# TianyiFranklinWang/MIRROR

Hardware: AMD Instinct MI355X
Metric: SSL samples/sec (slide+RNA pairs) (higher is better)
Workload: dtype bf16; 1 GPU; BASELINE c2: B=16/GPU x [4096 patch tokens x 1024-d] + [2048 genes], D=512, RNA depth 6 / 8 heads, train mode, local-batch InfoNCE; precision_policy=bf16, per_gpu_batch=16, global_batch=16, parallelism=dp1, grad_bucket_dtype=f32, step_launch=hip_graph

## Files before the change

### mirror_amd/csrc/gemm_big.hip

```cpp
#include "gemm_kernel.h"

static thread_local GemmTail g_tail = {nullptr, nullptr, 0, 0, 0, 0, 0, 0, 0, 0, 0.f};
GemmTail* gemm_pending_tail() { return &g_tail; }

namespace {

constexpr int BIG = 256, NTB = 512, BWM = 4, BWN = 2;

__device__ __forceinline__ f32x4 round_bf16_4(f32x4 x) {
    return f32x4{bf2f(f2bf(x[0])), bf2f(f2bf(x[1])), bf2f(f2bf(x[2])), bf2f(f2bf(x[3]))};
}
struct TileRow { int b0, t0, row0; };
template <int EPI>
__device__ __forceinline__ f32x4 epi_quad(const GemmArgs& g, f32x4 x, int grow, int gcol, const TileRow& tr) {
    if constexpr (EPI == MH_EPI_MASKPOS) {
        x = round_bf16_4(x);
        const int rpb = g.epi.rows_per_batch, first = g.epi.first;
        int t = tr.t0 + (grow - tr.row0), b = tr.b0;
        if (t >= rpb) { t -= rpb; b += 1; }
        if (t >= first && g.epi.mask[(long)b * (rpb - first) + (t - first)] != 0.f) x = *reinterpret_cast<const f32x4*>(g.epi.token + gcol);
        return x + *reinterpret_cast<const f32x4*>(g.epi.pos + (long)t * g.N + gcol);
    } else {
        return x;
    }
// ... 960 lines not shown
    __shared__ f32x4 red[PS > 1 ? 256 : 1];
    const int ql = threadIdx.x % QB, pg = threadIdx.x / QB;
    const long quads = mn / 4;
    for (long qb = blockIdx.x; qb * QB < quads; qb += gridDim.x) {
        const long q = qb * QB + ql;
        const bool live = q < quads;
        const long i = q * 4, r = live ? i / N : 0, c = live ? i % N : 0;
        f32x4 s = {0.f, 0.f, 0.f, 0.f};
        if (live) {
            int p = pg;
            for (; p + 7 * PS < parts; p += 8 * PS) {
                f32x4 v[8];
#pragma unroll
                for (int u = 0; u < 8; u++) v[u] = ld4_bf16(P + (long)(p + u * PS) * mn + i);
#pragma unroll
                for (int u = 0; u < 8; u++) s += v[u];
            }
            for (; p < parts; p += PS) s += ld4_bf16(P + (long)p * mn + i);
            if constexpr (TAIL) {
                f32x4 acc = {0.f, 0.f, 0.f, 0.f};
                const int total = t.batch * t.KT;
                auto ld = [&](int k, float& a, f32x4& b) {
                    const int z = k / t.KT, kk = k - z * t.KT;
                    const long ia = z * t.sA + (long)kk * t.lda + r, ib = z * t.sB + (long)kk * t.ldb + c;
                    a = t.a_f32 ? reinterpret_cast<const float*>(t.A)[ia] : bf2f(reinterpret_cast<const bf16_t*>(t.A)[ia]);
                    if (t.b_f32) b = *reinterpret_cast<const f32x4*>(reinterpret_cast<const float*>(t.B) + ib);
                    else {
                        const u32x2 w = *reinterpret_cast<const u32x2*>(reinterpret_cast<const bf16_t*>(t.B) + ib);
                        b = f32x4{__uint_as_float(w[0] << 16), __uint_as_float(w[0] & 0xffff0000u), __uint_as_float(w[1] << 16), __uint_as_float(w[1] & 0xffff0000u)};
                    }
                };
                int k = pg;
                for (; k + 7 * PS < total; k += 8 * PS) {
                    float a[8];
                    f32x4 b[8];
#pragma unroll
                    for (int u = 0; u < 8; u++) ld(k + u * PS, a[u], b[u]);
#pragma unroll
                    for (int u = 0; u < 8; u++) acc += b[u] * a[u];
                }
                for (; k < total; k += PS) {
                    float a;
                    f32x4 b;
                    ld(k, a, b);
                    acc += b * a;
                }
                s += acc * t.alpha;
            }
        }
        if constexpr (PS > 1) {
            __syncthreads();
            red[threadIdx.x] = s;
            __syncthreads();
            if (pg == 0 && live) {
#pragma unroll
                for (int u = 1; u < PS; u++) s += red[u * QB + ql];
            }
        }
        if (pg == 0 && live) {
            f32x4* cp = reinterpret_cast<f32x4*>(C + r * ldc + c);
            *cp = *cp + s;
        }
    }
}
static void launch_fold(const float* ws_, int parts, long mn, float* C, long ldc, int N, hipStream_t s) {
#ifdef MH_EXP
    if (getenv("MH_EXP_SKIP_FOLD")) { g_tail.KT = 0; return; }
#endif
    const bf16_t* ws = reinterpret_cast<const bf16_t*>(ws_);
    const long blocks1 = mh_cdiv(mn / 4, 256);
    const bool tail = g_tail.KT > 0 && (g_tail.ldb % 4) == 0 && (g_tail.sB % 4) == 0 && ((uintptr_t)g_tail.B & (g_tail.b_f32 ? 15 : 7)) == 0;
    const bool share = tail && blocks1 < 1024;
    const dim3 grid((unsigned)min(share ? mh_cdiv(mn / 4, 64) : blocks1, share ? 4096L : 2048L));
#define FOLD_(TAIL, PS) hipLaunchKernelGGL((fold_partials_kernel<TAIL, PS>), grid, dim3(256), 0, s, ws, parts, mn, C, ldc, N, g_tail)
    if (tail) {
        if (share) FOLD_(true, 4); else FOLD_(true, 1);
        g_tail.KT = 0;
    } else {
        FOLD_(false, 1);
    }
#undef FOLD_
}

static int pq_grid(long units) {
    static const int cus = [] { hipDeviceProp_t p; int d = 0; (void)hipGetDevice(&d); return hipGetDeviceProperties(&p, d) == hipSuccess ? p.multiProcessorCount : 256; }();
    return (int)(units < cus ? units : cus);
}
static int pq_variant(const GemmArgs& a, bool bf16_tiles, bool part, int epi) {
    const bool relu = a.act == MH_ACT_RELU;
    if (part) return a.alpha == 1.f ? 0 : 1;
    if (bf16_tiles) {
        if (a.accumulate || (epi != 0 && relu)) return -1;
        return relu ? 2 : (a.alpha == 1.f && !a.bias ? 0 : 1);
    }
    if (a.atomic || (epi != 0 && (relu || a.accumulate))) return -1;
    return a.accumulate ? (relu ? -1 : 2) : (relu ? 1 : 0);
}
template <typename K>
static void pp_attr(K kern) {
    (void)hipFuncSetAttribute(reinterpret_cast<const void*>(kern), hipFuncAttributeMaxDynamicSharedMemorySize, PP_LDS);
}
#define PQ_LAUNCH_VAR_(TC, AKC, BKC, PART, EPI, VAR, s, a, units_, grid)                                  \
    do {                                                                                             \
        static const bool attrq_ = (pp_attr(gemm_pq_kernel<TC, AKC, BKC, PART, EPI, VAR>), true);    \
        (void)attrq_;                                                                                \
        hipLaunchKernelGGL((gemm_pq_kernel<TC, AKC, BKC, PART, EPI, VAR>), dim3(pq_grid(units_)), dim3(NTB), PQ_LDS, s, a, (int)units_, \
                           (int)(grid).x, (int)(grid).y);                                            \
    } while (0)
#define PP_LAUNCH_(TC, AKC, BKC, PART, EPI, grid, s, a)                                              \
    do {                                                                                             \
        const int var_ = pq_variant(a, sizeof(TC) == 2, PART, EPI);                                  \
        const bool pq_ = !(a).shared_chip && var_ >= 0;                                              \
        gemm_note_variant("%s<%s,%s,%s%s%s>", pq_ ? "gemm_pq_kernel" : "gemm_pp_kernel", gemm_tn<TC>(), \
                          gemm_tf(AKC), gemm_tf(BKC), (PART) ? ",part" : "", (EPI) == 0 ? "" : ((EPI) == 1 ? ",epi1" : ((EPI) == 2 ? ",epi2" : ",epi3"))); \
        if (pq_) {                                                                                   \
            const long units_ = (long)(grid).x * (grid).y * (grid).z;                                \
            if (var_ == 0) PQ_LAUNCH_VAR_(TC, AKC, BKC, PART, EPI, 0, s, a, units_, grid);           \
            else if (var_ == 1) PQ_LAUNCH_VAR_(TC, AKC, BKC, PART, EPI, 1, s, a, units_, grid);      \
            else if constexpr ((EPI) == 0 && !(PART)) PQ_LAUNCH_VAR_(TC, AKC, BKC, PART, EPI, 2, s, a, units_, grid); \
        } else {                                                                                     \
            static const bool attr_ = (pp_attr(gemm_pp_kernel<TC, AKC, BKC, PART, EPI>), true);      \
            (void)attr_;                                                                             \
            hipLaunchKernelGGL((gemm_pp_kernel<TC, AKC, BKC, PART, EPI>), grid, dim3(NTB), PP_LDS, s, a); \
        }                                                                                            \
    } while (0)

template <typename TC>
void launch_big(GemmArgs& a, int akc, int bkc, int batch, hipStream_t s) {
    a.tiles_m = (a.M + BIG - 1) / BIG;
    a.tiles_n = a.N / BIG;
    dim3 grid(a.tiles_m * a.tiles_n, a.split_k, batch);
    const long parts = (long)a.split_k * batch, mn = (long)a.M * a.N;
    const bool partial = a.atomic && a.ws && a.M % BIG == 0 && a.ws_floats * 2 >= parts * mn && ((uintptr_t)a.ws & 15) == 0 && a.vecC &&
                         a.sC1 == 0 && a.sC2 == 0 && parts >= 8;
    if (!partial) a.ws = nullptr;
#define PP_DISPATCH_(PART)                                                             \
    do {                                                                               \
        if (akc && bkc) PP_LAUNCH_(TC, true, true, PART, 0, grid, s, a);               \
        else if (akc) PP_LAUNCH_(TC, true, false, PART, 0, grid, s, a);                \
        else if (bkc) PP_LAUNCH_(TC, false, true, PART, 0, grid, s, a);                \
        else PP_LAUNCH_(TC, false, false, PART, 0, grid, s, a);                        \
    } while (0)
    if constexpr (sizeof(TC) == 4) {
        if (partial) {
            PP_DISPATCH_(true);
            launch_fold((const float*)a.ws, (int)parts, mn, (float*)a.C, (long)a.ldc, a.N, s);
            return;
        }
    }
    PP_DISPATCH_(false);
#undef PP_DISPATCH_
}

}

bool gemm_try_big_fp8(GemmArgs& a, int dtC, int batch, hipStream_t s) {
    const bool ok = a.M > BIG && a.N % BIG == 0 && a.K % 64 == 0 && a.k_per_split == a.K && a.split_k == 1 && !a.atomic && !a.accumulate &&
                    a.vecA && a.vecB && a.vecC && !a.R && a.diag == 0.f && a.scale_a && a.scale_b;
    if (!ok || (long)((a.M + BIG - 1) / BIG) * (a.N / BIG) * batch < 128) return false;
    a.tiles_m = (a.M + BIG - 1) / BIG;
    a.tiles_n = a.N / BIG;
    dim3 grid(a.tiles_m * a.tiles_n, 1, batch);
    gemm_note_variant("gemm_big_kernel<%s,true,true,fp8>", dtC == MH_BF16 ? "bf16" : "float");
    if (dtC == MH_BF16) hipLaunchKernelGGL((gemm_big_kernel<bf16_t>), grid, dim3(NTB), 0, s, a);
    else hipLaunchKernelGGL((gemm_big_kernel<float>), grid, dim3(NTB), 0, s, a);
    return true;
}

const char* gemm_big_epi(GemmArgs& a, int akc, int bkc, int dtC, int batch, hipStream_t s) {
    if (!(akc && a.M > BIG && a.N % BIG == 0 && a.K % 64 == 0 && a.split_k == 1 && a.k_per_split == a.K && !a.atomic && !a.accumulate && !a.R &&
          a.diag == 0.f && a.vecA && a.vecB && a.vecC && batch == 1))
        return "shape is not on the 256 x 256 kernel (K-contiguous bf16 A, M > 256, N % 256 == 0, K % 64 == 0, one batch, no split-K / accumulate / R / diag)";
    if (a.a_rpb != 0 && a.a_rpb < BIG) return "a_rows_per_batch must be >= 256";
    if (a.ldc != a.N) return "C must be contiguous (ldc == N)";
    const mh_gemm_epi& e = a.epi;
    a.tiles_m = (a.M + BIG - 1) / BIG;
    a.tiles_n = a.N / BIG;
    dim3 grid(a.tiles_m * a.tiles_n, 1, 1);
#define EPI_LAUNCH_(TC, EPI) \
    do { if (bkc) PP_LAUNCH_(TC, true, true, false, EPI, grid, s, a); else PP_LAUNCH_(TC, true, false, false, EPI, grid, s, a); } while (0)
    switch (e.kind) {
    case MH_EPI_DROPADD:
        if (dtC != MH_F32 || !e.resid || !(e.p >= 0.f && e.p < 1.f) || (e.offset & 7) || ((uintptr_t)e.resid & 15)) return "DROPADD: f32 C, a 16-byte aligned residual, 0 <= p < 1, offset % 8 == 0";
        EPI_LAUNCH_(float, MH_EPI_DROPADD);
        return nullptr;
    case MH_EPI_MASKPOS:
        if (dtC != MH_F32 || !e.mask || !e.token || !e.pos || e.rows_per_batch < BIG || e.first < 0) return "MASKPOS: f32 C, mask / token / pos, rows_per_batch >= 256";
        if (((uintptr_t)e.token & 15) || ((uintptr_t)e.pos & 15)) return "MASKPOS: token / pos must be 16-byte aligned";
        EPI_LAUNCH_(float, MH_EPI_MASKPOS);
        return nullptr;
    case MH_EPI_SQERR:
        if (dtC != MH_BF16 || !e.mask || !e.tgt || !e.sq || e.rows_per_batch <= 0 || e.rows_per_batch % BIG || a.M % e.rows_per_batch || a.act != MH_ACT_NONE) return "SQERR: bf16 C, mask / tgt / sq, rows_per_batch % 256 == 0";
        if (((uintptr_t)e.tgt & 15) || e.tgt_bs % 4) return "SQERR: tgt must be 16-byte aligned";
        EPI_LAUNCH_(bf16_t, MH_EPI_SQERR);
        return nullptr;
// ... 32 lines not shown
```

### mirror_amd/functional.py

```python
from __future__ import annotations

from dataclasses import dataclass
from typing import List, Optional, Tuple

import os

import torch
from torch.autograd import Function

from . import kernels as K
from ._lib import ACT_NONE, ACT_RELU, MH_BF16, MH_F32

f32, bf16 = torch.float32, torch.bfloat16


@dataclass(frozen=True)
class Precision:
    name: str
    mma: int
    act: torch.dtype
    pinv_mma: int
    fp8_fwd: bool = False


# ... 1542 lines not shown
        dz_new = K.gemm(dz, tr(T3), alpha=0.25, mma=pm, out_dtype=f32)
        dP = K.gemm(dT3, tr(T2), alpha=-1.0, mma=pm, out_dtype=f32)
        dT2 = K.gemm(tr(P), dT3, alpha=-1.0, mma=pm, out_dtype=f32)
        K.gemm(dT2, tr(P), out=dP, accumulate=True, R=dT2, rcoef=-7.0, mma=pm)
        K.gemm(tr(P), dT2, out=dP, accumulate=True, mma=pm)
        K.gemm(dP, tr(z), out=dX, accumulate=True, mma=pm)
        K.gemm(tr(a2), dP, out=dz_new, accumulate=True, mma=pm)
        dz = dz_new
    z0 = saved[0][0]
    K.pinv_z0_bwd(a2, K.cast(z0, f32), dz, st, dX)
    return dX


def pinv_forward_tile(a2: torch.Tensor, iters: int, want_a2b: bool = False):
    st = K.pinv_absmax(a2, zeros((4,), a2.device).view(torch.int64))
    a2b = K.cast(a2, bf16)
    zs = torch.empty((iters + 1,) + tuple(a2.shape), device=a2.device, dtype=bf16)
    pt = torch.empty((iters, 2) + tuple(a2.shape), device=a2.device, dtype=bf16)
    K.cast(K.pinv_z0(a2, st), bf16, out=zs[0])
    saved = []
    for k in range(iters):
        z, P, T2 = zs[k], pt[k, 1], pt[k, 0]
        K.gemm(a2b, z, P, mma=MH_BF16)
        K.gemm(P, P, T2, diag=15.0, R=P, rcoef=-7.0, mma=MH_BF16)
        T3 = K.gemm(P, T2, alpha=-1.0, diag=13.0, mma=MH_BF16)
        K.gemm(z, T3, zs[k + 1], alpha=0.25, mma=MH_BF16)
        saved.append((z, P, T2, T3))
    if want_a2b:
        return zs[iters], saved, st, a2b
    return zs[iters], saved, st


_TILE_SIDE = True
_PINV_R32 = True


def pinv_backward_tile(a2, saved, st, dZ, a2b=None):
    tr = lambda t: t.transpose(-1, -2)
    iters = len(saved)
    if a2b is None:
        a2b = K.cast(a2, bf16)
    dz = K.cast(dZ, bf16) if dZ.dtype != bf16 else dZ
    dzn = dZ
    z0 = saved[0][0]
    stacked = (iters > 1 and saved[1][0].data_ptr() - z0.data_ptr() == z0.numel() * 2
               and saved[0][1].data_ptr() - saved[0][2].data_ptr() == z0.numel() * 2)
    dPs = torch.empty((iters,) + tuple(a2.shape), device=a2.device, dtype=bf16)
    dd = torch.empty((2,) + tuple(a2.shape), device=a2.device, dtype=bf16)
    for k in range(iters - 1, -1, -1):
        z, P, T2, T3 = saved[k]
        nT3, dT2, dPb = dd[0], dd[1], dPs[k]
        K.gemm(tr(z), dz, nT3, alpha=-0.25, mma=MH_BF16)
        dzn = K.gemm(dz, tr(T3), alpha=0.25, mma=MH_BF16, out_dtype=f32)
        K.gemm(tr(P), nT3, dT2, mma=MH_BF16)
        if stacked:
            dP = K.gemm_ksum(dd, tr(_pair(T2, P)), R=dT2, rcoef=-7.0, mma=MH_BF16, out_dtype=f32)
        else:
            dP = K.gemm(nT3, tr(T2), mma=MH_BF16, out_dtype=f32)
            K.gemm(dT2, tr(P), out=dP, accumulate=True, R=dT2, rcoef=-7.0, mma=MH_BF16)
        if _PINV_R32:
            K.gemm(tr(P), dT2, out=dPb, R=dP, rcoef=1.0, mma=MH_BF16)
        else:
            K.gemm(tr(P), dT2, out=dP, accumulate=True, mma=MH_BF16, c2=dPb)
        dz = torch.empty(dzn.shape, device=dzn.device, dtype=bf16)
        if _PINV_R32 and k > 0:
            K.gemm(tr(a2b), dPb, out=dz, R=dzn, rcoef=1.0, mma=MH_BF16)
        else:
            K.gemm(tr(a2b), dPb, out=dzn, accumulate=True, mma=MH_BF16, c2=dz)
    if stacked:
        zst = torch.as_strided(z0, (iters,) + tuple(z0.shape), (z0.numel(),) + tuple(z0.stride()))
        dX = K.gemm_ksum(dPs, tr(zst), mma=MH_BF16, out_dtype=f32)
    else:
        dX = torch.zeros_like(a2)
        for k in range(iters):
            K.gemm(dPs[k], tr(saved[k][0]), out=dX, accumulate=True, mma=MH_BF16)
    K.pinv_z0_bwd(a2, None, dzn, st, dX)
    return dX


def _pair(first: torch.Tensor, second: torch.Tensor) -> torch.Tensor:
    return torch.as_strided(first, (2,) + tuple(first.shape), (first.numel(),) + tuple(first.stride()))


_SIM2_MASKED = True
_RC_FUSED = True


class NystromCoreFn(Function):

    @staticmethod
    def forward(ctx, qkv, res_w, heads, l, iters, prec, kmask=None, q8_key=None, lm_ext=None, link=None, q8_out=None):
        qkv = qkv.contiguous()
        Bn, n_p, D3 = qkv.shape
        D, h = D3 // 3, heads
        dh = D // h
        A, mma, pm = prec.act, prec.mma, prec.pinv_mma
        scale = dh ** -0.5
        q, k, v = (_heads(qkv, i, 3, h) for i in range(3))
        if lm_ext is not None:
            lm = lm_ext if K._lm_ld(lm_ext) > 0 else lm_ext.contiguous()
        else:
            lm = K.landmark_fwd(qkv, l)
        ctx.lm_ext = lm_ext is not None
        if kmask is not None:
            mrow, mlm, lscale = kmask
            if lscale is not None:
                lm = K.row_scale(lm if lm.is_contiguous() else lm.contiguous(), lscale)
        ql, kl = _heads(lm, 0, 2, h), _heads(lm, 1, 2, h)
        m_l = lm.shape[1]
        chain = pm == MH_BF16 and m_l == K.PINV_CHAIN_M
        one = chain and (kmask is None or _SIM2_MASKED) and dh == 64 and K.nys_sim2_ok(lm, h)
        mlm_s2 = None if kmask is None else mlm
        if one:
            a2, xt = K.nys_sim2_alloc(lm, h)
            st = zeros((4,), qkv.device).view(torch.int64)
        else:
            a2 = K.gemm(ql, kl.transpose(-1, -2), alpha=scale, mma=mma, out_dtype=f32)
            if kmask is None:
                K.softmax_fwd(a2, a2)
            else:
                K.softmax_masked_fwd(a2, mlm, mlm, a2)
        sd = f32 if pm == MH_F32 else bf16
        side = None
        if chain:
            chain_saved = K.pinv_chain_saved_alloc(iters, Bn * h, m_l, qkv.device)
            z0 = None
            if not one:
                st = K.pinv_absmax(a2, zeros((4,), a2.device).view(torch.int64))
                z0, xt = K.pinv_chain_prep(a2, st, K.pinv_chain_z0_slot(chain_saved))
            zfT = torch.empty((Bn, h, m_l, m_l), device=qkv.device, dtype=bf16)
            zf = zfT.transpose(-1, -2)
            side = _side_stream(qkv.device)
            side.wait_stream(torch.cuda.current_stream())
            with torch.cuda.stream(side):
                if one:
                    K.nys_sim2(lm, h, scale, st, out=(a2, xt), mlm=mlm_s2)
                    K.pinv_chain_fwd(xt, chain_saved, zfT, iters, z0f=a2, stats=st, z0_rowmajor=True)
                else:
                    K.pinv_chain_fwd(xt, chain_saved, zfT, iters)
            saved = [(xt, chain_saved, z0 if z0 is not None else st)]
            ctx.z0_stored = z0 is not None
            K.shared_chip = True
        tile = (not chain) and pm == MH_BF16 and K.gemm_tile_ok(m_l, m_l, m_l)
        if tile and _TILE_SIDE:
            side = _side_stream(qkv.device)
            side.wait_stream(torch.cuda.current_stream())
            with torch.cuda.stream(side):
                zf, saved, st, ctx.a2b = pinv_forward_tile(a2, iters, want_a2b=True)
        if link is not None:
            link.core = True
            link.run("v_cols")
        fused = K.nys_fused_ok(qkv, h, m_l) and lm.dtype == bf16
        lse1 = lse3 = a1 = a3 = None
        out = torch.empty((Bn, n_p, D), device=qkv.device, dtype=A)
        rc_in_a3 = fused and _RC_FUSED and A == bf16 and res_w.numel() == h * 33
        if fused:
            av, lse3 = K.nys_attn3_fwd(qkv, lm, h, scale, kmask,
                                       rc=(res_w.detach().reshape(-1).contiguous(), out) if rc_in_a3 else None)
        else:
            sm1 = (kmask is None and A == bf16 and mma == MH_BF16 and q.dtype == bf16
                   and K.gemm_softmax_ok(n_p, lm.shape[1], dh, q.dtype, kl.dtype))
            if sm1:
                a1 = K.gemm(q, kl.transpose(-1, -2), alpha=scale, mma=mma, out_dtype=bf16, softmax=True)
            else:
                a1 = K.gemm(q, kl.transpose(-1, -2), alpha=scale, mma=mma, out_dtype=f32)
            a3 = K.gemm(ql, k.transpose(-1, -2), alpha=scale, mma=mma, out_dtype=f32)
            if kmask is None:
                if not sm1:
                    a1 = K.softmax_fwd(a1, a1 if A == f32 else None, out_dtype=A)
                a3 = K.softmax_fwd(a3, a3 if A == f32 else None, out_dtype=A)
            else:
                a1 = K.softmax_masked_fwd(a1, mrow, mlm, a1 if A == f32 else None, out_dtype=A)
                a3 = K.softmax_masked_fwd(a3, mlm, mrow, a3 if A == f32 else None, out_dtype=A)
        if tile and not _TILE_SIDE:
            zf, saved, st, ctx.a2b = pinv_forward_tile(a2, iters, want_a2b=True)
        elif not chain and not tile:
            zf, saved, st = pinv_forward(a2, iters, pm, sd)
        if not fused:
            av = K.gemm(a3, v, mma=mma, out_dtype=f32)
        pio = pm if (pm == MH_BF16 or A == f32) else mma
        w2 = None
        if side is not None and fused:
            w2 = torch.empty((Bn, h, m_l, dh), device=qkv.device, dtype=A)
            av_ready = torch.cuda.current_stream().record_event()
            with torch.cuda.stream(side):
                side.wait_event(av_ready)
                K.gemm(zf, av, out=w2, mma=pio)
        if fused and not rc_in_a3:
            K.resconv(qkv[..., 2 * D:], res_w.detach().contiguous(), out, h, transpose=False, accumulate=False)
        if side is not None:
            torch.cuda.current_stream().wait_stream(side)
            if chain:
                K.shared_chip = False
        if w2 is None:
            w2 = K.gemm(zf, av, mma=pio, out_dtype=A)
        o1 = None
        if fused:
            o1 = torch.empty_like(out)
            st8 = _fp8_state
            site = st8["sites"].get(q8_key) if (q8_key is not None and st8["tick"] is not None and kmask is None) else None
            if site is not None and st8["host_step"] - site[1] >= 2:
                q8 = torch.empty(out.shape, device=out.device, dtype=torch.uint8)
                lse1, sc8 = K.nys_attn1_fwd_q8(qkv, lm, w2, out, h, scale, True, q8, site[0], st8["tick"], o1=o1)
                q8_out.append((q8, sc8))
            else:
                lse1 = K.nys_attn1_fwd(qkv, lm, w2, out, h, scale, accumulate=True, kmask=kmask, o1=o1)
        else:
            K.gemm(a1, w2, out=_heads(out, 0, 1, h), mma=mma)
            K.resconv(qkv[..., 2 * D:], res_w.detach().contiguous(), out, h, transpose=False, accumulate=True)
        stats = (lse1, lse3) if fused else (a1, a3)
        if link is not None and link.capture is not None:
            link.capture.update(qkv=qkv, lm=lm, z=zfT if chain else (zf if zf.dtype == f32 else K.cast(zf, f32)), z_colmajor=bool(chain),
                                lse3=lse3 if fused else None, kmask=kmask, heads=h, scale=scale)
        ctx.has_o1 = o1 is not None
        ctx.save_for_backward(qkv, res_w, lm, stats[0], a2, stats[1], av, w2, st, zfT if chain else zf,
                              *([o1] if o1 is not None else []), *[t for it in saved for t in it])
        ctx.cfg = (heads, l, prec)
        ctx.chain = (chain, iters, fused)
        ctx.tile = tile
        ctx.kmask, ctx.link = kmask, link
        return out

    @staticmethod
    def backward(ctx, dout):
        qkv, res_w, lm, a1, a2, a3, av, w2, st, zf, *flat = ctx.saved_tensors
        o1 = None
        if ctx.has_o1:
            o1, flat = flat[0], flat[1:]
        chain, iters, fused = ctx.chain
        kmask = ctx.kmask
        if kmask is not None:
            mrow, mlm, lscale = kmask
        sm_bwd = (lambda y, dy, rm, cm: K.softmax_bwd(y, dy)) if kmask is None else K.softmax_masked_bwd
        zfT = zf if chain else None
        if chain:
            zf = zf.transpose(-1, -2)
        saved = None if chain else [tuple(flat[i:i + 4]) for i in range(0, len(flat), 4)]
        heads, l, prec = ctx.cfg
        A, mma, pm = prec.act, prec.mma, prec.pinv_mma
        Bn, n_p, D3 = qkv.shape
        D, h = D3 // 3, heads
        dh = D // h
        m = n_p // l
        scale = dh ** -0.5
        tr = lambda t: t.transpose(-1, -2)
        dout = dout.contiguous()
        if dout.dtype != A:
            dout = K.cast(dout, A)
        q, k, v = (_heads(qkv, i, 3, h) for i in range(3))
        ql, kl = _heads(lm, 0, 2, h), _heads(lm, 1, 2, h)
        dO = _heads(dout, 0, 1, h)
        de = dlm_out = None
        if ctx.lm_ext and A == bf16:
            de, dqkv, dlm_out = ext_rows_alloc(Bn, n_p, m, D3, 2 * D, qkv.device)
        else:
            dqkv = torch.empty_like(qkv)
        dq, dk, dv = (_heads(dqkv, i, 3, h) for i in range(3))
        rw = res_w.detach().contiguous()
        dres, dres_sunk = _gbuf(res_w, (rw.numel(),))
        if fused:
            lse1, lse3 = a1, a3
            dW2 = zeros((Bn, h, m, dh), qkv.device)
            dlm = zeros((Bn, m, 2 * D), qkv.device)
            delta1 = torch.empty_like(lse1)
            K.nys_attn1_bwd(qkv, lm, w2, dout, lse1, o1, delta1, dqkv, dW2, dlm, h, scale, kmask)
        else:
            dW2 = K.gemm(tr(a1), dO, mma=mma, out_dtype=f32)
            dlm = torch.empty((Bn, m, 2 * D), device=qkv.device, dtype=f32)
        dql, dkl = _heads(dlm, 0, 2, h), _heads(dlm, 1, 2, h)
        sd = f32 if pm == MH_F32 else bf16
        pio = pm if (pm == MH_BF16 or A == f32) else mma
        one2 = (chain and fused and A == bf16 and pio == MH_BF16 and dh == 64 and m == 256 and dW2.dtype == f32 and av.dtype == f32)
        dAV = dzb = None
        if one2:
            dzb, dAV = K.nys_dz_dav(dW2, av.contiguous(), zfT)
        else:
            dZ = K.gemm(dW2, tr(av), mma=pm, out_dtype=bf16 if (ctx.tile and _PINV_R32 and iters >= 1) else f32)
        side = dlm2 = None
        if chain:
            xb, chain_saved, z0 = flat
            work = K.pinv_chain_work_alloc(iters, Bn * h, m, qkv.device)
            dS2 = torch.empty_like(a2)
            dz0 = torch.empty_like(a2)
            if dzb is None:
                dzb = K.pinv_chain_pack(dZ)
            if fused and (kmask is None or _SIM2_MASKED):
                dlm2 = torch.empty_like(dlm)
            side = _side_stream(qkv.device)
            side.wait_stream(torch.cuda.current_stream())
            with torch.cuda.stream(side):
                K.pinv_chain_bwd(xb, chain_saved, dzb, work, dS2, dz0, iters)
                if (kmask is None or _SIM2_MASKED) and not ctx.z0_stored and a2.shape[-1] == 256:
                    K.pinv_s2_bwd(a2, dz0, st, dS2, _zeroed1(a2.device), mlm=mlm if kmask else None, heads=h)
                else:
                    K.pinv_z0_bwd(a2, z0 if ctx.z0_stored else None, dz0, st, dS2, _zeroed1(a2.device))
                    sm_bwd(a2, dS2, mlm if kmask else None, mlm if kmask else None)
                if dlm2 is not None:
                    K.gemm(tr(dS2), ql, out=_heads(dlm2, 1, 2, h), alpha=scale, mma=pio)
                    K.gemm(dS2, kl, out=_heads(dlm2, 0, 2, h), alpha=scale, mma=pio)
            K.shared_chip = True
        tile_side = ctx.tile and _TILE_SIDE and not chain
        if tile_side:
            dZ_ready = torch.cuda.current_stream().record_event()
            side = _side_stream(qkv.device)
            with torch.cuda.stream(side):
                side.wait_event(dZ_ready)
                dS2 = pinv_backward_tile(a2, saved, st, dZ, getattr(ctx, "a2b", None))
                sm_bwd(a2, dS2, mlm if kmask else None, mlm if kmask else None)
        if ctx.link is not None:
            ctx.link.run("wgrad")
        rc_bwd_one = fused and _RC_FUSED and A == bf16
        if not rc_bwd_one:
            K.resconv_wgrad(qkv[..., 2 * D:], dout, dres, h)
        if dAV is None:
            dAV = K.gemm(tr(zf), dW2, mma=pio, out_dtype=A)
        if fused:
            K.nys_attn3_bwd(qkv, lm, av, dAV, lse3, dqkv, dlm, h, scale, kmask)
            if rc_bwd_one:
                K.resconv_bwd(dout, qkv[..., 2 * D:], rw, dqkv[..., 2 * D:], dres, h)
            else:
                K.resconv(dout, rw, dqkv[..., 2 * D:], h, transpose=True, accumulate=True)
        else:
            if (kmask is None and A == bf16 and mma == MH_BF16 and a1.dtype == bf16 and a1.is_contiguous()
                    and K.gemm_softmax_ok(n_p, m, dh, dO.dtype, w2.dtype)):
                dS1 = K.gemm(dO, tr(w2), mma=mma, out_dtype=bf16, softmax_bwd_of=a1)
            else:
                dS1 = K.gemm(dO, tr(w2), mma=mma, out_dtype=A)
                sm_bwd(a1, dS1, mrow if kmask else None, mlm if kmask else None)
            dS3 = K.gemm(dAV, tr(v), mma=mma, out_dtype=A)
            K.gemm(tr(a3), dAV, out=dv, mma=mma)
            K.resconv(dout, rw, dqkv[..., 2 * D:], h, transpose=True, accumulate=True)
            sm_bwd(a3, dS3, mlm if kmask else None, mrow if kmask else None)
            K.gemm(dS1, kl, out=dq, alpha=scale, mma=mma)
            K.gemm(tr(dS3), ql, out=dk, alpha=scale, mma=mma)
            K.gemm(tr(dS1), q, out=dkl, alpha=scale, mma=mma)
            K.gemm(dS3, k, out=dql, alpha=scale, mma=mma)
        if tile_side:
            torch.cuda.current_stream().wait_stream(side)
        elif side is not None:
            torch.cuda.current_stream().wait_stream(side)
            K.shared_chip = False
            del work
        else:
            dS2 = pinv_backward_tile(a2, saved, st, dZ, getattr(ctx, "a2b", None)) if ctx.tile else pinv_backward(a2, saved, st, dZ, pm, sd)
            sm_bwd(a2, dS2, mlm if kmask else None, mlm if kmask else None)
        if dlm2 is None:
            K.gemm(tr(dS2), ql, out=dkl, alpha=scale, accumulate=True, mma=pio)
            K.gemm(dS2, kl, out=dql, alpha=scale, accumulate=True, mma=pio)
        dres = _gret(res_w, dres, dres_sunk)
        dres = None if dres is None else dres.view_as(res_w)
        if de is not None and ctx.link is not None and (kmask is None or (lscale is None and dlm2 is not None)):
            merge = lambda: K.lm_merge(dlm, dlm2, de[Bn * n_p:], D3 - 2 * D)
            ctx.link.lm_merge = (de, merge)
            return dqkv, dres, None, None, None, None, None, None, dlm_out, None, None
        if dlm2 is not None:
            dlm = K.add(dlm, dlm2, out_dtype=A)
        if kmask is not None and lscale is not None:
            dlm = K.row_scale(dlm, lscale)
        if ctx.lm_ext:
            if de is not None:
                dlm_out.copy_(dlm)
                de[Bn * n_p:, 2 * D:].zero_()
                return dqkv, dres, None, None, None, None, None, None, dlm_out, None, None
            return dqkv, dres, None, None, None, None, None, None, dlm, None, None
        K.landmark_bwd(K.cast(dlm, A), dqkv, l)
        return dqkv, dres, None, None, None, None, None, None, None, None, None


class RowScaleFn(Function):

    @staticmethod
    def forward(ctx, x, s):
        ctx.save_for_backward(s)
        return K.row_scale(x.contiguous(), s)

    @staticmethod
    def backward(ctx, dy):
        (s,) = ctx.saved_tensors
        return K.row_scale(dy.contiguous(), s), None


_PROBE = os.environ.get("MIRROR_PROBE", "0") != "0"
_probe_names: List[str] = []
_probe_buf: Optional[torch.Tensor] = None


def probe(name: str) -> None:
    global _probe_buf
    if not _PROBE:
        return
    if _probe_buf is None:
        _probe_buf = torch.zeros(256, dtype=torch.int64, device="cuda")
    if name not in _probe_names:
        _probe_names.append(name)
    K.timestamp(_probe_buf[_probe_names.index(name):_probe_names.index(name) + 1])


def probe_read() -> dict:
    torch.cuda.synchronize()
    v = _probe_buf[:len(_probe_names)].tolist()
    return dict(zip(_probe_names, v))


class ProbeFn(Function):

    @staticmethod
    def forward(ctx, x, name):
        ctx.name = name
        probe(name + ".fwd")
        return x.view_as(x)

    @staticmethod
    def backward(ctx, g):
        probe(ctx.name + ".bwd")
        return g, None


def probe_point(x: torch.Tensor, name: str) -> torch.Tensor:
    if not (_PROBE and x.requires_grad):
        return x
    y = ProbeFn.apply(x, name)
    for attr in ("_bf16", "_relu_slot", "_drop_site", "_fan_slot"):
        if getattr(x, attr, None) is not None:
            setattr(y, attr, getattr(x, attr))
# ... 636 lines not shown
```

### mirror_amd/kernels.py

```python
from __future__ import annotations

import ctypes as C
import functools
import os
from typing import Optional


import torch

from . import _lib
from ._lib import ACT_GELU, ACT_NONE, ACT_RELU, MH_BF16, MH_F32, GemmDesc, MirrorHipError

_DT = {torch.float32: MH_F32, torch.bfloat16: MH_BF16}


def dt(t: torch.Tensor) -> int:
    try:
        return _DT[t.dtype]
    except KeyError:
        raise MirrorHipError(f"unsupported dtype {t.dtype} (f32 / bf16 only)") from None


_raw_stream = getattr(torch._C, "_cuda_getCurrentRawStream", None)

# ... 54 lines not shown
    nd = max(a.dim(), b.dim())
    a4, a_rm, lda, sa1, sa2 = _mat(a)
    b4, b_rm, ldb, sb1, sb2 = _mat(b)
    M, K = a4.shape[2], a4.shape[3]
    K2, N = b4.shape[2], b4.shape[3]
    if K != K2:
        raise MirrorHipError(f"gemm: inner dims differ: {tuple(a.shape)} @ {tuple(b.shape)}")
    B1 = max(a4.shape[0], b4.shape[0])
    B2 = max(a4.shape[1], b4.shape[1])
    for t4 in (a4, b4):
        if t4.shape[0] not in (1, B1) or t4.shape[1] not in (1, B2):
            raise MirrorHipError(f"gemm: batch dims do not broadcast: {tuple(a.shape)} @ {tuple(b.shape)}")
    if a4.dtype != b4.dtype and mma == MH_F32:
        raise MirrorHipError(f"gemm: f32 MMA needs f32 operands, got {a4.dtype} x {b4.dtype}")
    if out is None:
        if accumulate:
            raise MirrorHipError("gemm: accumulate needs an explicit output")
        out = torch.empty((B1, B2, M, N), device=a.device, dtype=out_dtype or a.dtype)
        o4 = out
        out = out.reshape(out.shape[4 - nd:])
    else:
        o4 = out
        while o4.dim() < 4:
            o4 = o4.unsqueeze(0)
        if tuple(o4.shape) != (B1, B2, M, N):
            raise MirrorHipError(f"gemm: output shape {tuple(out.shape)} != {(B1, B2, M, N)}")
    so = o4.stride()
    if not (so[3] == 1 or N == 1):
        raise MirrorHipError("gemm: output must have unit stride in its last dim")
    if mma == MH_F32 and (a4.dtype != torch.float32 or b4.dtype != torch.float32 or o4.dtype != torch.float32):
        raise MirrorHipError("gemm: f32 MMA needs f32 operands and output")
    if bias is not None:
        if bias.dtype != torch.float32 or bias.numel() != N or not bias.is_contiguous():
            raise MirrorHipError("gemm: bias must be contiguous f32 [N]")
    d = GemmDesc()
    d.A, d.B, d.C, d.bias = a4.data_ptr(), b4.data_ptr(), o4.data_ptr(), _p(bias)
    d.M, d.N, d.K = M, N, K
    d.lda, d.ldb, d.ldc = lda, ldb, (so[2] if M > 1 else max(N, 1))
    d.a_kc, d.b_kc = int(a_rm), int(not b_rm)
    d.dtA, d.dtB, d.dtC, d.mma = dt(a4), dt(b4), dt(o4), mma
    d.batch1, d.batch2 = B1, B2
    d.sA1, d.sA2, d.sB1, d.sB2 = sa1, sa2, sb1, sb2
    d.sC1, d.sC2 = (so[0] if B1 > 1 else 0), (so[1] if B2 > 1 else 0)
    d.alpha, d.diag, d.act, d.accumulate, d.split_k = alpha, diag, act, int(accumulate), max(1, int(split_k))
    if R is not None:
        _chk(R)
        tile = gemm_tile_ok(M, N, K, a4.dtype, b4.dtype) and bias is None and act == ACT_NONE and d.split_k == 1
        if R.numel() != o4.numel() or tuple(R.stride()) != tuple(out.stride()) or not (
                R.dtype == o4.dtype or (tile and R.dtype in (torch.bfloat16, torch.float32))):
            raise MirrorHipError("gemm: R must have the output's dtype (or bf16 / f32 on the 192 x 384 tile kernel), shape and strides")
        d.R, d.rcoef = R.data_ptr(), rcoef
        d.r_bf16 = 0 if R.dtype == o4.dtype else (1 if R.dtype == torch.bfloat16 else 2)
    if c2 is not None:
        _chk(c2)
        if c2.dtype != torch.bfloat16 or c2.numel() != o4.numel() or tuple(c2.stride()) != tuple(out.stride()):
            raise MirrorHipError("gemm: c2 must be a bf16 tensor with the output's shape and strides")
        d.C2 = c2.data_ptr()
    if softmax:
        if not (gemm_softmax_ok(M, N, K, a4.dtype, b4.dtype) and o4.dtype == torch.bfloat16 and bias is None and act == ACT_NONE
                and d.split_k == 1 and not accumulate and R is None and c2 is None and diag == 0.0):
            raise MirrorHipError("gemm: softmax=True needs bf16 operands and output, M % 192 == 0, N == 384, K % 8 == 0 and a plain product")
        d.row_softmax = 1
    if softmax_bwd_of is not None:
        P_ = softmax_bwd_of
        _chk(P_)
        if not (gemm_softmax_ok(M, N, K, a4.dtype, b4.dtype) and o4.dtype == torch.bfloat16 and P_.dtype == torch.bfloat16 and bias is None
                and act == ACT_NONE and d.split_k == 1 and not accumulate and R is None and c2 is None and diag == 0.0 and not softmax
                and P_.numel() == o4.numel() and tuple(P_.stride()) == tuple(out.stride())):
            raise MirrorHipError("gemm: softmax_bwd_of needs bf16 operands / output / probabilities (same layout as out), M % 192 == 0, N == 384")
        d.row_softmax, d.R = 2, P_.data_ptr()
    if kseg is not None and int(kseg[0]) > 1:
        if not (gemm_tile_ok(M, N, K, a4.dtype, b4.dtype) and bias is None and act == ACT_NONE and d.split_k == 1):
            raise MirrorHipError("gemm: a sum over operand pairs (kseg) needs the 192 x 384 tile kernel (see gemm_tile_ok)")
        d.k_segments, d.sA_seg, d.sB_seg = int(kseg[0]), int(kseg[1]), int(kseg[2])
    wsb = int(_lib.load().mh_gemm_workspace_bytes(C.byref(d))) if (accumulate and SPLITK_PARTIALS == "bf16") else 0
    if 0 < wsb <= (1 << 29):
        ws = torch.empty((wsb // 4,), device=a.device, dtype=torch.float32)
        d.workspace, d.workspace_floats = ws.data_ptr(), ws.numel()
    d.shared_chip = int(shared_chip)
    _launch_gemm(d)
    return out


shared_chip = False


EPI_DROPADD, EPI_MASKPOS, EPI_SQERR = 1, 2, 3
_EPI_ON = True


def linear_fused_ok(x: torch.Tensor, w: torch.Tensor, window: Optional[tuple] = None) -> bool:
    if not (_EPI_ON and x.dtype == torch.bfloat16 and w.dtype == torch.bfloat16 and x.dim() == 3 and x.is_contiguous() and w.dim() == 2
            and w.is_contiguous() and x.is_cuda):
        return False
    Bn, T, Kd = x.shape
    R = T if window is None else window[1]
    return (w.shape[1] == Kd and Kd % 64 == 0 and w.shape[0] % 256 == 0 and Bn * R > 256 and (window is None or R >= 256 or Bn == 1)
            and x.data_ptr() % 16 == 0 and w.data_ptr() % 16 == 0)


def linear_fused_tail(rows: int) -> int:
    rem = rows % 256
    return rem if (rows > 512 and 0 < rem <= 64) else 0


def linear_fused(x: torch.Tensor, w: torch.Tensor, bias: Optional[torch.Tensor], out: torch.Tensor, epi: "_lib.GemmEpi",
                 window: Optional[tuple] = None, m_rows: Optional[int] = None) -> torch.Tensor:
    _chk(x, w, out, bias)
    Bn, T, Kd = x.shape
    r0, R = (0, T) if window is None else window
    N = w.shape[0]
    if not out.is_contiguous() or out.numel() != Bn * R * N:
        raise MirrorHipError("linear_fused: out must be contiguous [B * R, N]")
    d = GemmDesc()
    d.A, d.B, d.C, d.bias = x.data_ptr() + r0 * Kd * 2, w.data_ptr(), out.data_ptr(), _p(bias)
    d.M, d.N, d.K = (Bn * R if m_rows is None else int(m_rows)), N, Kd
    d.lda, d.ldb, d.ldc = Kd, Kd, N
    d.a_kc, d.b_kc = 1, 1
    d.dtA, d.dtB, d.dtC, d.mma = MH_BF16, MH_BF16, dt(out), MH_BF16
    d.batch1 = d.batch2 = 1
    d.alpha, d.split_k = 1.0, 1
    if R != T and Bn > 1:
        d.a_rows_per_batch, d.a_row_skip = R, T - R
    d.epi = C.pointer(epi)
    _launch_gemm(d)
    return out


def _weight_view_ld(b2: torch.Tensor, who: str) -> tuple:
    if b2.stride(0) == 1:
        return b2.stride(1), 1
    if b2.stride(1) == 1:
        return b2.stride(0), 0
    raise MirrorHipError(f"{who}: the weight view must have a unit stride")


def gemm_rows_window(a3: torch.Tensor, b2: torch.Tensor, out3: torch.Tensor, r0: int, R: int, m_rows: Optional[int] = None,
                     a_r0: Optional[int] = None) -> None:
    _chk(a3, b2, out3)
    Bn, Ta, Kd = a3.shape
    T = out3.shape[1]
    N = b2.shape[1]
    bf = torch.bfloat16
    a_r0 = r0 if a_r0 is None else a_r0
    if not (a3.dtype == b2.dtype == out3.dtype == bf and a3.stride(2) == 1 and out3.stride(2) == 1 and a3.stride(0) == Ta * a3.stride(1)
            and out3.stride(0) == T * out3.stride(1) and tuple(out3.shape) == (Bn, T, N) and b2.shape[0] == Kd and 0 <= r0 and r0 + R <= T
            and 0 <= a_r0 and a_r0 + R <= Ta):
        raise MirrorHipError("gemm_rows_window: bad operands")
    d = GemmDesc()
    d.A, d.B, d.C, d.bias = a3.data_ptr() + a_r0 * a3.stride(1) * 2, b2.data_ptr(), out3.data_ptr() + r0 * out3.stride(1) * 2, None
    d.M, d.N, d.K = (Bn * R if m_rows is None else int(m_rows)), N, Kd
    d.lda, d.ldc = a3.stride(1), out3.stride(1)
    d.ldb, d.b_kc = _weight_view_ld(b2, "gemm_rows_window")
    d.a_kc = 1
    d.dtA, d.dtB, d.dtC, d.mma = MH_BF16, MH_BF16, MH_BF16, MH_BF16
    d.batch1 = d.batch2 = 1
    d.alpha, d.split_k = 1.0, 1
    if Bn > 1:
        if R != Ta:
            d.a_rows_per_batch, d.a_row_skip = R, Ta - R
        if R != T:
            d.c_rows_per_batch, d.c_row_skip = R, T - R
    d.shared_chip = 1 if shared_chip else 0
    _launch_gemm(d)


def gemm_rows_ext_ok(Bn: int, T: int, r0: int, R: int, extra: int, Kd: int, N: int, a2: torch.Tensor, out2: torch.Tensor) -> bool:
    bf = torch.bfloat16
    M = Bn * R + extra
    return (a2.dim() == 2 and out2.dim() == 2 and a2.dtype == bf and out2.dtype == bf and a2.is_cuda and R >= 256 and M > 512 and 0 <= extra < R
            and r0 + R == T and M % 256 <= extra
            and N % 256 == 0 and Kd % 64 == 0 and a2.stride(1) == 1 and out2.stride(1) == 1 and a2.stride(0) % 8 == 0 and out2.stride(0) % 8 == 0
            and a2.data_ptr() % 16 == 0 and out2.data_ptr() % 16 == 0 and a2.shape[0] == Bn * T + extra and out2.shape[0] == Bn * T + extra)


def gemm_rows_ext(a2: torch.Tensor, b2: torch.Tensor, out2: torch.Tensor, Bn: int, T: int, r0: int, R: int, extra: int) -> int:
    _chk(a2, b2, out2)
    Kd, N = a2.shape[1], b2.shape[1]
    if not gemm_rows_ext_ok(Bn, T, r0, R, extra, Kd, N, a2, out2) or b2.shape[0] != Kd or b2.dtype != torch.bfloat16:
        raise MirrorHipError("gemm_rows_ext: bad operands")
    M = Bn * R + extra
    tail = M % 256
    d = GemmDesc()
    d.A, d.B, d.C, d.bias = a2.data_ptr() + r0 * a2.stride(0) * 2, b2.data_ptr(), out2.data_ptr() + r0 * out2.stride(0) * 2, None
    d.M, d.N, d.K = M - tail, N, Kd
    d.lda, d.ldc = a2.stride(0), out2.stride(0)
    d.ldb, d.b_kc = _weight_view_ld(b2, "gemm_rows_ext")
    d.a_kc = 1
    d.dtA, d.dtB, d.dtC, d.mma = MH_BF16, MH_BF16, MH_BF16, MH_BF16
    d.batch1 = d.batch2 = 1
    d.alpha, d.split_k = 1.0, 1
    if R != T:
        d.a_rows_per_batch, d.a_row_skip = R, T - R
        d.c_rows_per_batch, d.c_row_skip = R, T - R
        d.window_batches = Bn
    d.shared_chip = 1 if shared_chip else 0
    _launch_gemm(d)
    return tail


def gemm_rows_window_ok(a3: torch.Tensor, out3: torch.Tensor, r0: int, R: int, N: int) -> bool:
    bf = torch.bfloat16
    return (a3.dim() == 3 and out3.dim() == 3 and a3.dtype == bf and out3.dtype == bf and a3.is_cuda and R >= 256 and a3.shape[0] * R > 512
            and N % 256 == 0 and a3.shape[2] % 64 == 0 and a3.stride(2) == 1 and out3.stride(2) == 1 and a3.stride(1) % 8 == 0
            and out3.stride(1) % 8 == 0 and a3.data_ptr() % 16 == 0 and out3.data_ptr() % 16 == 0
            and a3.stride(0) == a3.shape[1] * a3.stride(1) and out3.stride(0) == out3.shape[1] * out3.stride(1))


def epi_dropadd(resid: torch.Tensor, p: float, seed: int, offset: int, dev_base) -> "_lib.GemmEpi":
    _chk(resid)
    e = _lib.GemmEpi()
    e.kind, e.resid, e.p, e.seed, e.offset, e.dev_base = EPI_DROPADD, resid.data_ptr(), float(p), int(seed), int(offset), _p(dev_base)
    return e


def epi_maskpos(mask: torch.Tensor, token: torch.Tensor, pos: torch.Tensor, rows_per_batch: int, first: int) -> "_lib.GemmEpi":
    _chk(mask, token, pos)
    e = _lib.GemmEpi()
    e.kind, e.mask, e.token, e.pos, e.rows_per_batch, e.first = EPI_MASKPOS, mask.data_ptr(), token.data_ptr(), pos.data_ptr(), int(rows_per_batch), int(first)
    return e


def epi_sqerr(mask: torch.Tensor, tgt: torch.Tensor, tgt_bs: int, sq: torch.Tensor, rows_per_batch: int) -> "_lib.GemmEpi":
    _chk(mask, tgt, sq)
    e = _lib.GemmEpi()
    e.kind, e.mask, e.tgt, e.tgt_bs, e.sq, e.rows_per_batch = EPI_SQERR, mask.data_ptr(), tgt.data_ptr(), int(tgt_bs), sq.data_ptr(), int(rows_per_batch)
    return e


def gemm_softmax_ok(M: int, N: int, Kd: int, dta=torch.bfloat16, dtb=torch.bfloat16) -> bool:
    return M % 192 == 0 and N == 384 and Kd % 8 == 0 and dta == torch.bfloat16 and dtb == torch.bfloat16


def gemm_ksum(a_stack: torch.Tensor, b_stack: torch.Tensor, out: Optional[torch.Tensor] = None, **kw) -> torch.Tensor:
    if a_stack.shape[0] != b_stack.shape[0] or a_stack.shape[0] < 1:
        raise MirrorHipError("gemm_ksum: the stacks need the same, non-zero leading length")
    return gemm(a_stack[0], b_stack[0], out, kseg=(a_stack.shape[0], a_stack.stride(0), b_stack.stride(0)), **kw)


def gemm_tile_ok(M: int, N: int, Kd: int, dta=torch.bfloat16, dtb=torch.bfloat16) -> bool:
    return M % 192 == 0 and N % 384 == 0 and Kd % 64 == 0 and dta == torch.bfloat16 and dtb == torch.bfloat16


import os as _os
SPLITK_PARTIALS = _os.environ.get("MIRROR_SPLITK_PARTIALS", "bf16")
if SPLITK_PARTIALS not in ("bf16", "f32"):
    raise MirrorHipError(f"MIRROR_SPLITK_PARTIALS={SPLITK_PARTIALS!r}: 'bf16' or 'f32'")


class GemmProfiler:

    def __init__(self, only: Optional[str] = None):
        self.only = only
        self.records = []

    def launch(self, d: GemmDesc, fn) -> None:
        if torch.cuda.is_current_stream_capturing():
            fn()
            return
        e0, e1 = torch.cuda.Event(enable_timing=True), torch.cuda.Event(enable_timing=True)
        e0.record()
        fn()
        e1.record()
        name = (_lib.load().mh_gemm_variant_name() or b"").decode()
        if d.epi and not name.endswith(f",epi{d.epi.contents.kind}>"):
            name = name[:-1] + f",epi{d.epi.contents.kind}>"
        self.records.append((name, 2.0 * d.M * d.N * d.K * d.batch1 * d.batch2, e0, e1))

    def launch_named(self, v: str, flops: float, fn) -> None:
        if (self.only is not None and v != self.only) or torch.cuda.is_current_stream_capturing():
            fn()
            return
        e0, e1 = torch.cuda.Event(enable_timing=True), torch.cuda.Event(enable_timing=True)
        e0.record()
        fn()
        e1.record()
        self.records.append((v, flops, e0, e1))

    def summary(self):
# ... 1859 lines not shown
```

Before: 2167 samples/s.

## Cap persistent GEMM grid to CUs left free by concurrent pinv chain

While the pseudo-inverse chain kernel runs on a side stream, GEMMs used to fall back to the non-persistent pp kernel whenever shared_chip was set. The flag now carries a workgroup budget equal to the CU count minus the chain's workgroups, rounded down to a multiple of 8. The persistent pq kernel is used with its grid capped to that budget, so the two streams can overlap without competing for CUs. If the budget is below 8 it becomes 1 and the old fallback path is kept. The risk is a wrong budget estimate, which could leave CUs idle or still cause contention.

```diff
diff --git a/mirror_amd/csrc/gemm_big.hip b/mirror_amd/csrc/gemm_big.hip
--- a/mirror_amd/csrc/gemm_big.hip
+++ b/mirror_amd/csrc/gemm_big.hip
@@ -1066,9 +1066,11 @@
 #undef FOLD_
 }
 
-static int pq_grid(long units) {
+static int pq_grid(long units, int shared_chip) {
     static const int cus = [] { hipDeviceProp_t p; int d = 0; (void)hipGetDevice(&d); return hipGetDeviceProperties(&p, d) == hipSuccess ? p.multiProcessorCount : 256; }();
-    return (int)(units < cus ? units : cus);
+    int wgs = cus;
+    if (shared_chip >= 8 && (shared_chip & ~7) < cus) wgs = shared_chip & ~7;
+    return (int)(units < wgs ? units : wgs);
 }
 static int pq_variant(const GemmArgs& a, bool bf16_tiles, bool part, int epi) {
     const bool relu = a.act == MH_ACT_RELU;
@@ -1088,13 +1090,13 @@
     do {                                                                                             \
         static const bool attrq_ = (pp_attr(gemm_pq_kernel<TC, AKC, BKC, PART, EPI, VAR>), true);    \
         (void)attrq_;                                                                                \
-        hipLaunchKernelGGL((gemm_pq_kernel<TC, AKC, BKC, PART, EPI, VAR>), dim3(pq_grid(units_)), dim3(NTB), PQ_LDS, s, a, (int)units_, \
+        hipLaunchKernelGGL((gemm_pq_kernel<TC, AKC, BKC, PART, EPI, VAR>), dim3(pq_grid(units_, (a).shared_chip)), dim3(NTB), PQ_LDS, s, a, (int)units_, \
                            (int)(grid).x, (int)(grid).y);                                            \
     } while (0)
 #define PP_LAUNCH_(TC, AKC, BKC, PART, EPI, grid, s, a)                                              \
     do {                                                                                             \
         const int var_ = pq_variant(a, sizeof(TC) == 2, PART, EPI);                                  \
-        const bool pq_ = !(a).shared_chip && var_ >= 0;                                              \
+        const bool pq_ = ((a).shared_chip == 0 || (a).shared_chip >= 8) && var_ >= 0;                \
         gemm_note_variant("%s<%s,%s,%s%s%s>", pq_ ? "gemm_pq_kernel" : "gemm_pp_kernel", gemm_tn<TC>(), \
                           gemm_tf(AKC), gemm_tf(BKC), (PART) ? ",part" : "", (EPI) == 0 ? "" : ((EPI) == 1 ? ",epi1" : ((EPI) == 2 ? ",epi2" : ",epi3"))); \
         if (pq_) {                                                                                   \
diff --git a/mirror_amd/functional.py b/mirror_amd/functional.py
--- a/mirror_amd/functional.py
+++ b/mirror_amd/functional.py
@@ -1648,6 +1648,14 @@
     return torch.as_strided(first, (2,) + tuple(first.shape), (first.numel(),) + tuple(first.stride()))
 
 
+_CHAIN_BUDGET_FWD = None
+_CHAIN_BUDGET_BWD = None
+
+
+def _chain_budget(hook, chain_wgs: int, device) -> int:
+    return K.chain_budget(chain_wgs, device) if hook is None else int(hook)
+
+
 _SIM2_MASKED = True
 _RC_FUSED = True
 
@@ -1706,7 +1714,7 @@
                     K.pinv_chain_fwd(xt, chain_saved, zfT, iters)
             saved = [(xt, chain_saved, z0 if z0 is not None else st)]
             ctx.z0_stored = z0 is not None
-            K.shared_chip = True
+            K.shared_chip = _chain_budget(_CHAIN_BUDGET_FWD, Bn * h, qkv.device)
         tile = (not chain) and pm == MH_BF16 and K.gemm_tile_ok(m_l, m_l, m_l)
         if tile and _TILE_SIDE:
             side = _side_stream(qkv.device)
@@ -1757,7 +1765,7 @@
         if side is not None:
             torch.cuda.current_stream().wait_stream(side)
             if chain:
-                K.shared_chip = False
+                K.shared_chip = 0
         if w2 is None:
             w2 = K.gemm(zf, av, mma=pio, out_dtype=A)
         o1 = None
@@ -1864,7 +1872,7 @@
                 if dlm2 is not None:
                     K.gemm(tr(dS2), ql, out=_heads(dlm2, 1, 2, h), alpha=scale, mma=pio)
                     K.gemm(dS2, kl, out=_heads(dlm2, 0, 2, h), alpha=scale, mma=pio)
-            K.shared_chip = True
+            K.shared_chip = _chain_budget(_CHAIN_BUDGET_BWD, Bn * h, qkv.device)
         tile_side = ctx.tile and _TILE_SIDE and not chain
         if tile_side:
             dZ_ready = torch.cuda.current_stream().record_event()
@@ -1905,7 +1913,7 @@
             torch.cuda.current_stream().wait_stream(side)
         elif side is not None:
             torch.cuda.current_stream().wait_stream(side)
-            K.shared_chip = False
+            K.shared_chip = 0
             del work
         else:
             dS2 = pinv_backward_tile(a2, saved, st, dZ, getattr(ctx, "a2b", None)) if ctx.tile else pinv_backward(a2, saved, st, dZ, pm, sd)
diff --git a/mirror_amd/kernels.py b/mirror_amd/kernels.py
--- a/mirror_amd/kernels.py
+++ b/mirror_amd/kernels.py
@@ -160,7 +160,13 @@
     return out
 
 
-shared_chip = False
+shared_chip = 0
+
+
+def chain_budget(chain_wgs: int, device=None) -> int:
+    free = (torch.cuda.get_device_properties(device if device is not None else torch.cuda.current_device()).multi_processor_count
+            - int(chain_wgs)) & ~7
+    return free if free >= 8 else 1
 
 
 EPI_DROPADD, EPI_MASKPOS, EPI_SQERR = 1, 2, 3
@@ -201,6 +207,7 @@
     if R != T and Bn > 1:
         d.a_rows_per_batch, d.a_row_skip = R, T - R
     d.epi = C.pointer(epi)
+    d.shared_chip = int(shared_chip)
     _launch_gemm(d)
     return out
 
@@ -239,7 +246,7 @@
             d.a_rows_per_batch, d.a_row_skip = R, Ta - R
         if R != T:
             d.c_rows_per_batch, d.c_row_skip = R, T - R
-    d.shared_chip = 1 if shared_chip else 0
+    d.shared_chip = int(shared_chip)
     _launch_gemm(d)
 
 
@@ -272,7 +279,7 @@
         d.a_rows_per_batch, d.a_row_skip = R, T - R
         d.c_rows_per_batch, d.c_row_skip = R, T - R
         d.window_batches = Bn
-    d.shared_chip = 1 if shared_chip else 0
+    d.shared_chip = int(shared_chip)
     _launch_gemm(d)
     return tail
 
```

Result: no change. 2169 samples/s (median of 3 runs) (+0.1%).
